# tiborcamargo/KinectPy

Hardware: AMD Instinct MI355X
Metric: Mpoints/sec end-to-end (unproject+filter+ICP), 4-sensor frame (higher is better)
Workload: dtype f64 decisions / f32 storage

## Files before the change

### kinectpy_amd/csrc/kpx_voxel.hip

```cpp
#include "kpx_voxelsteps.h"

namespace kpx {

template <bool NRM>
__global__ __launch_bounds__(256) void voxel_mean_kernel(StoredLoad load, int64_t n, const int32_t *__restrict__ vals, const int32_t *__restrict__ seg_start,
                                                         int32_t *__restrict__ d_count, const int32_t *__restrict__ err, float *__restrict__ opts,
                                                         float *__restrict__ ocol, float *__restrict__ onrm)
{
    const int32_t m_total = *d_count;
    if (blockIdx.x == 0 && threadIdx.x == 0 && *err) *d_count = KPX_ERR_RANGE;
    for (int64_t m = (int64_t)blockIdx.x * blockDim.x + threadIdx.x; m < m_total; m += (int64_t)gridDim.x * blockDim.x) {
        const int64_t s0 = seg_start[m], s1 = (m + 1 < m_total) ? seg_start[m + 1] : n;
        double sp[3] = { 0, 0, 0 }, sc[3] = { 0, 0, 0 }, sn[3] = { 0, 0, 0 };
        voxel_segment_sum<NRM>(vals, s0, s1, load, sp, sc, sn);
        voxel_write_row(sp, sc, (double)(s1 - s0), opts + 3 * m, (load.col && ocol) ? ocol + 3 * m : nullptr);
        if (NRM && onrm) {
            double nn = sqrt(fma(sn[2], sn[2], fma(sn[1], sn[1], sn[0] * sn[0])));
#pragma unroll
            for (int a = 0; a < 3; ++a) onrm[3 * m + a] = (float)(nn > 0 ? sn[a] / nn : sn[a]);
        }
    }
}
static int voxel_impl(const float *pts, const float *col, const float *nrm, int64_t n, double voxel, float *opts,
                      float *ocol, float *onrm, int32_t *d_count, Arena &a, hipStream_t st)
{
    VoxelScratch s;
    voxel_carve(a, n, kPlainCarve, &s);
    KPX_ARENA_CHECK(a);
    int rc = bbox_f32(pts, n, s.bbox, s.part, st);
    if (rc) return rc;
    KPX_HIP(hipMemsetAsync(s.err, 0, sizeof(int32_t), st));
    int nb = (int)(cdiv(n, 256) > 4096 ? 4096 : cdiv(n, 256));
    CloudSet<1> one;
    one.pts[0] = pts; one.off[0] = 0; one.off[1] = n; one.count = 1;
    hipLaunchKernelGGL((voxel_key_kernel<CloudSet<1>, StoredPoint, FixedKeys>), dim3(nb), dim3(256), 0, st, one, (const double *)s.bbox, voxel,
                       FixedKeys{ s.sort.keys_in, s.err }, s.sort.vals_in);
    rc = voxel_sort_and_heads<uint64_t>(s, n, 63, d_count, st);
    if (rc) return rc;
    const StoredLoad load = { pts, col, nrm, 0 };
    const auto mean_kernel = nrm ? &voxel_mean_kernel<true> : &voxel_mean_kernel<false>;
    hipLaunchKernelGGL(mean_kernel, dim3(nb), dim3(256), 0, st, load, n, (const int32_t *)s.sort.vals_out,
                       (const int32_t *)s.seg_start, d_count, (const int32_t *)s.err, opts, ocol, onrm);
    KPX_LAUNCH_CHECK();
    return KPX_OK;
}

constexpr int kVoxelBatchMax = 8;
constexpr int kVoxelBatchBboxBlocks = 64;
constexpr VoxelCarve kBatchCarve = { kVoxelBatchMax, kVoxelBatchBboxBlocks, true, true, 64 };
struct VoxelBatch : CloudSet<kVoxelBatchMax> {
    const float *col[kVoxelBatchMax];
    float *opts[kVoxelBatchMax];
    float *ocol[kVoxelBatchMax];
    int32_t morton;
};
static VoxelBatch voxel_batch_of(const float *const *h_pts, const float *const *h_col, const int64_t *h_n, float *const *h_opts, float *const *h_ocol,
                                 int first, int count, bool morton)
{
    VoxelBatch b;
    b.count = count;
    b.morton = morton ? 1 : 0;
    b.off[0] = 0;
    for (int i = 0; i < kVoxelBatchMax; ++i) {
        const bool on = i < count;
        b.pts[i] = on ? h_pts[first + i] : nullptr;
        b.col[i] = (on && h_col) ? h_col[first + i] : nullptr;
        b.opts[i] = on ? h_opts[first + i] : nullptr;
        b.ocol[i] = (on && h_col && h_ocol) ? h_ocol[first + i] : nullptr;
        b.off[i + 1] = b.off[i] + (on ? h_n[first + i] : 0);
    }
    return b;
}
__device__ __forceinline__ void voxel_batch_axis_bits(const double d[3], int bits[3])
{
#pragma unroll
    for (int a = 0; a < 3; ++a) {
        const unsigned long long m = (unsigned long long)d[a] - 1ull;
        int n = 1;
        while (n < 21 && (m >> n) != 0ull) ++n;
        bits[a] = n;
    }
}
__device__ __forceinline__ unsigned long long voxel_hcode(unsigned long long x, unsigned long long y, unsigned long long z, int bits)
{
    unsigned long long X[3] = { x, y, z };
    const unsigned long long M = 1ull << (bits - 1);
    for (unsigned long long Q = M; Q > 1ull; Q >>= 1) {
        const unsigned long long P = Q - 1ull;
#pragma unroll
        for (int i = 0; i < 3; ++i) {
            if (X[i] & Q) X[0] ^= P;
            else { const unsigned long long t = (X[0] ^ X[i]) & P; X[0] ^= t; X[i] ^= t; }
        }
    }
    X[1] ^= X[0];
    X[2] ^= X[1];
    unsigned long long t = 0ull;
    for (unsigned long long Q = M; Q > 1ull; Q >>= 1)
        if (X[2] & Q) t ^= Q - 1ull;
    X[0] ^= t; X[1] ^= t; X[2] ^= t;
    unsigned long long k = 0ull;
    for (int b = bits - 1; b >= 0; --b) {
#pragma unroll
        for (int i = 0; i < 3; ++i) k = (k << 1) | ((X[i] >> b) & 1ull);
    }
    return k;
}
__device__ __forceinline__ int voxel_hilbert_cube_bits(const int ab[3], int cb)
{
    const int top = ab[0] > ab[1] ? (ab[0] > ab[2] ? ab[0] : ab[2]) : (ab[1] > ab[2] ? ab[1] : ab[2]);
    const int low = ab[0] < ab[1] ? (ab[0] < ab[2] ? ab[0] : ab[2]) : (ab[1] < ab[2] ? ab[1] : ab[2]);
    const int passes = (ab[0] + ab[1] + ab[2] + cb + 7) / 8;
    for (int m = top; m > low; --m) {
        int n = 3 * m + cb;
#pragma unroll
        for (int a = 0; a < 3; ++a) n += ab[a] > m ? ab[a] - m : 0;
        if (n <= 64 && (n + 7) / 8 <= passes) return m;
    }
    return low;
}
__device__ __forceinline__ int voxel_hilbert_key_bits(const int ab[3], int m)
{
    int n = 3 * m;
#pragma unroll
    for (int a = 0; a < 3; ++a) n += ab[a] > m ? ab[a] - m : 0;
    return n;
}
__device__ __forceinline__ unsigned long long voxel_hilbert_key(unsigned long long x, unsigned long long y, unsigned long long z, const int ab[3], int m)
{
    const unsigned long long mask = (1ull << m) - 1ull;
    const int ey = ab[1] > m ? ab[1] - m : 0, ez = ab[2] > m ? ab[2] - m : 0;
    const unsigned long long hi = (((x >> m) << ey | (y >> m)) << ez) | (z >> m);
    return (hi << (3 * m)) | voxel_hcode(x & mask, y & mask, z & mask, m);
}
__device__ __forceinline__ void voxel_batch_dims(const VoxelBatch &b, const double *__restrict__ bbox, double voxel, double d[3], int *overflow)
{
    d[0] = d[1] = d[2] = 1.0;
    for (int c = 0; c < b.count; ++c) {
        if (b.off[c + 1] == b.off[c]) continue;
        double f[3];
        (void)voxel_cell(bbox + 8 * c + 3, bbox + 8 * c, voxel, f);
        for (int a = 0; a < 3; ++a) {
            const double e = f[a] + 1.0;
            if (e > d[a] && e < kVoxelAxisCells) d[a] = e;
        }
    }
    *overflow = ((double)b.count * d[0]) * (d[1] * d[2]) >= 18446744073709551616.0 ? 1 : 0;
}
__device__ __forceinline__ int voxel_batch_key_bits(const VoxelBatch &b, const double d[3], int overflow)
{
    int n = 64;
    if (!overflow && b.morton) {
        int cb = 0, ab[3];
        while ((1 << cb) < b.count) ++cb;
        voxel_batch_axis_bits(d, ab);
        n = voxel_hilbert_key_bits(ab, voxel_hilbert_cube_bits(ab, cb)) + cb;
        n = n < 1 ? 1 : (n > 64 ? 64 : n);
    } else if (!overflow) {
        const unsigned long long range = (((unsigned long long)b.count * (unsigned long long)d[0]) * (unsigned long long)d[1]) * (unsigned long long)d[2];
        n = 1;
        while (n < 64 && (range >> n) != 0ull) ++n;
    }
    return n;
}
__global__ void voxel_batch_bits_kernel(VoxelBatch b, const double *__restrict__ bbox, double voxel, int32_t *__restrict__ bits)
{
    double d[3];
    int overflow;
    voxel_batch_dims(b, bbox, voxel, d, &overflow);
    *bits = voxel_batch_key_bits(b, d, overflow);
}
template <class Key> struct BatchKeys {
    struct Grid {
        uint64_t DX, DY, DZ;
        int overflow, morton, ab[3], m;
    };
    Key *keys;
    int32_t *err, *bits_out;
    __device__ __forceinline__ Grid grid(const VoxelBatch &b, const double *__restrict__ bbox, double voxel) const
    {
        __shared__ double dims[3];
        __shared__ int overflow, axis_bits[3], cube_bits;
        if (threadIdx.x == 0) {
            double d[3];
            int ov;
            voxel_batch_dims(b, bbox, voxel, d, &ov);
            if (bits_out && blockIdx.x == 0) *bits_out = voxel_batch_key_bits(b, d, ov);
            dims[0] = d[0]; dims[1] = d[1]; dims[2] = d[2];
            int ab[3], cb = 0;
            voxel_batch_axis_bits(d, ab);
            axis_bits[0] = ab[0]; axis_bits[1] = ab[1]; axis_bits[2] = ab[2];
            while ((1 << cb) < b.count) ++cb;
            cube_bits = voxel_hilbert_cube_bits(ab, cb);
            overflow = (ov || (b.morton && voxel_hilbert_key_bits(ab, cube_bits) + cb > 64)) ? 1 : 0;
        }
        __syncthreads();
        return Grid{ (uint64_t)dims[0], (uint64_t)dims[1], (uint64_t)dims[2], overflow, b.morton, { axis_bits[0], axis_bits[1], axis_bits[2] }, cube_bits };
    }
    __device__ __forceinline__ void put(const Grid &g, const double *__restrict__ bbox, double voxel, int64_t i, int c, const double q[3]) const
    {
        double f[3];
        const bool bad = voxel_cell(q, bbox + 8 * c, voxel, f) || g.overflow;
        if (bad) { err[c] = 1; f[0] = f[1] = f[2] = 0.0; }
        if (g.morton)
            keys[i] = (Key)(((uint64_t)c << voxel_hilbert_key_bits(g.ab, g.m)) | voxel_hilbert_key((uint64_t)f[0], (uint64_t)f[1], (uint64_t)f[2], g.ab, g.m));
        else keys[i] = (Key)((((uint64_t)c * g.DX + (uint64_t)f[0]) * g.DY + (uint64_t)f[1]) * g.DZ + (uint64_t)f[2]);
    }
};
__global__ __launch_bounds__(64) void voxel_batch_locate_kernel(VoxelBatch b, const int32_t *__restrict__ seg_start, const int32_t *__restrict__ d_total,
                                                                const int32_t *__restrict__ err, int32_t *__restrict__ head, int32_t *__restrict__ d_counts)
{
    __shared__ int32_t h[kVoxelBatchMax + 1];
    const int c = threadIdx.x;
    const int32_t m = *d_total;
    if (c <= b.count) {
        int32_t lo = 0, hi = m;
        const int64_t want = b.off[c];
        while (lo < hi) {
            const int32_t mid = lo + (hi - lo) / 2;
            if (seg_start[mid] < want) lo = mid + 1; else hi = mid;
        }
        h[c] = c == b.count ? m : lo;
        head[c] = h[c];
    }
    __syncthreads();
    if (c < b.count) d_counts[c] = err[c] ? KPX_ERR_RANGE : h[c + 1] - h[c];
}
__global__ __launch_bounds__(256) void voxel_batch_mean_kernel(VoxelBatch b, const int32_t *__restrict__ vals, const int32_t *__restrict__ seg_start,
                                                               const int32_t *__restrict__ d_total, const int32_t *__restrict__ head)
{
    const int32_t m_total = *d_total;
    const int64_t total = b.off[b.count];
    for (int64_t m = (int64_t)blockIdx.x * blockDim.x + threadIdx.x; m < m_total; m += (int64_t)gridDim.x * blockDim.x) {
        const int64_t s0 = seg_start[m], s1 = (m + 1 < m_total) ? seg_start[m + 1] : total;
        const int c = b.cloud_of(s0);
        const StoredLoad load = { b.pts[c], b.col[c], nullptr, b.off[c] };
        double sp[3] = { 0, 0, 0 }, sc[3] = { 0, 0, 0 }, sn[3];
        voxel_segment_sum<false>(vals, s0, s1, load, sp, sc, sn);
        const int64_t o = m - head[c];
        voxel_write_row(sp, sc, (double)(s1 - s0), b.opts[c] + 3 * o, (load.col && b.ocol[c]) ? b.ocol[c] + 3 * o : nullptr);
    }
}

static int voxel_batch_impl(const VoxelBatch &b, double voxel, int32_t *d_counts, Arena &a, hipStream_t st, int spec_bits = 0,
                            int32_t *d_bits = nullptr)
{
    const int64_t total = b.off[b.count];
    VoxelScratch s;
    voxel_carve(a, total, kBatchCarve, &s);
    KPX_ARENA_CHECK(a);
    BoxDst boxes;
    for (int c = 0; c < kVoxelBatchMax; ++c) boxes.box[c] = s.bbox + 8 * c;
    boxes.err = s.err;
    hipLaunchKernelGGL((cloud_bbox_partial_kernel<VoxelBatch, StoredPoint, float, kVoxelBatchBboxBlocks>), dim3(kVoxelBatchBboxBlocks, b.count), dim3(256), 0, st, b, s.part);
    hipLaunchKernelGGL(cloud_bbox_final_kernel<kVoxelBatchBboxBlocks>, dim3(b.count), dim3(64), 0, st, (const double *)s.part, boxes);
    const int nb = (int)(cdiv(total, 256) > 4096 ? 4096 : cdiv(total, 256));
    int end_bit = 64;
    int32_t *bits_out = nullptr;
    if (spec_bits > 0 && d_bits) {
        bits_out = d_bits;
        end_bit = spec_bits > 64 ? 64 : spec_bits;
    } else if (total > (int64_t)128 * 1024) {
        int32_t *h_bits = static_cast<int32_t *>(thread_resources().pinned(kPinVoxelBits, sizeof(int32_t)));
        if (!h_bits) return KPX_ERR_HIP;
        hipLaunchKernelGGL(voxel_batch_bits_kernel, dim3(1), dim3(1), 0, st, b, s.bbox, voxel, s.head);
        KPX_HIP(hipMemcpyAsync(h_bits, s.head, sizeof(int32_t), hipMemcpyDeviceToHost, st));
        if (d_bits) KPX_HIP(hipMemcpyAsync(d_bits, s.head, sizeof(int32_t), hipMemcpyDefault, st));
        KPX_HIP(hipStreamSynchronize(st));
        end_bit = *h_bits < 1 ? 1 : (*h_bits > 64 ? 64 : *h_bits);
    } else if (d_bits) {
        hipLaunchKernelGGL(voxel_batch_bits_kernel, dim3(1), dim3(1), 0, st, b, s.bbox, voxel, d_bits);
    }
    int rc;
    if (end_bit <= 32) {
        hipLaunchKernelGGL((voxel_key_kernel<VoxelBatch, StoredPoint, BatchKeys<uint32_t>>), dim3(nb), dim3(256), 0, st, b, (const double *)s.bbox, voxel,
                           BatchKeys<uint32_t>{ reinterpret_cast<uint32_t *>(s.sort.keys_in), s.err, bits_out }, s.sort.vals_in);
        rc = voxel_sort_and_heads<uint32_t>(s, total, end_bit, s.d_total, st);
    } else {
        hipLaunchKernelGGL((voxel_key_kernel<VoxelBatch, StoredPoint, BatchKeys<uint64_t>>), dim3(nb), dim3(256), 0, st, b, (const double *)s.bbox, voxel,
                           BatchKeys<uint64_t>{ s.sort.keys_in, s.err, bits_out }, s.sort.vals_in);
        rc = voxel_sort_and_heads<uint64_t>(s, total, end_bit, s.d_total, st);
    }
    if (rc) return rc;
    hipLaunchKernelGGL(voxel_batch_locate_kernel, dim3(1), dim3(64), 0, st, b, s.seg_start, s.d_total, s.err, s.head, d_counts);
    hipLaunchKernelGGL(voxel_batch_mean_kernel, dim3(nb), dim3(256), 0, st, b, s.sort.vals_out, s.seg_start, s.d_total, s.head);
    KPX_LAUNCH_CHECK();
    return KPX_OK;
}

constexpr int kFuseMax = 16;
constexpr int kFuseBboxBlocks = 32;
constexpr VoxelCarve kFuseCarve = { kFuseMax, kFuseBboxBlocks, false, true, 63 };
struct FuseBatch : CloudSet<kFuseMax> {
    const float *col[kFuseMax];
    double T[kFuseMax][12];
    const double *dT[kFuseMax];
};
__global__ __launch_bounds__(64) void fuse_bbox_final_kernel(const double *__restrict__ part, int rows, double *__restrict__ bbox, int32_t *__restrict__ err)
{
    const int lane = lane_id();
    double v[6] = { INFINITY, INFINITY, INFINITY, -INFINITY, -INFINITY, -INFINITY };
    for (int r = lane; r < rows; r += 64) {
#pragma unroll
        for (int a = 0; a < 3; ++a) { v[a] = fmin(v[a], part[(int64_t)r * 6 + a]); v[3 + a] = fmax(v[3 + a], part[(int64_t)r * 6 + 3 + a]); }
    }
    box_wave_fold(v, v + 3);
    if (lane == 0) {
        for (int a = 0; a < 6; ++a) bbox[a] = v[a];
        *err = 0;
    }
}
__device__ __forceinline__ int fuse_key_bits(const double *__restrict__ bbox, double voxel, double d[3], bool *sane_out)
{
    (void)voxel_cell(bbox + 3, bbox, voxel, d);
#pragma unroll
    for (int a = 0; a < 3; ++a) d[a] += 1.0;
    const bool sane = d[0] >= 1.0 && d[1] >= 1.0 && d[2] >= 1.0 && d[0] < kVoxelAxisCells && d[1] < kVoxelAxisCells && d[2] < kVoxelAxisCells;
    int bits = 64;
    if (sane && d[0] * d[1] * d[2] < 18446744073709551616.0) {
        const unsigned long long range = (unsigned long long)d[0] * (unsigned long long)d[1] * (unsigned long long)d[2];
        bits = 1;
        while (bits < 64 && (range >> bits) != 0ull) ++bits;
    }
    *sane_out = sane;
    return bits;
}
__global__ void fuse_bits_kernel(const double *__restrict__ bbox, double voxel, int32_t *__restrict__ bits_out)
{
    double d[3];
    bool sane;
    *bits_out = fuse_key_bits(bbox, voxel, d, &sane);
}
struct ExtentKeys32 {
    struct Grid {
        double d[3];
        unsigned long long DY, DZ;
    };
    uint32_t *keys;
    int32_t *bits_out;
    template <class Set> __device__ __forceinline__ Grid grid(const Set &, const double *__restrict__ bbox, double voxel) const
    {
        Grid g;
        bool sane;
        const int bits = fuse_key_bits(bbox, voxel, g.d, &sane);
        if (blockIdx.x == 0 && threadIdx.x == 0) *bits_out = bits;
        g.DY = sane ? (unsigned long long)g.d[1] : 1ull;
        g.DZ = sane ? (unsigned long long)g.d[2] : 1ull;
        return g;
    }
    __device__ __forceinline__ void put(const Grid &g, const double *__restrict__ bbox, double voxel, int64_t i, int, const double q[3]) const
    {
        double f[3];
        if (voxel_cell(q, bbox, voxel, f, g.d)) f[0] = f[1] = f[2] = 0.0;
        keys[i] = (uint32_t)(((unsigned long long)f[0] * g.DY + (unsigned long long)f[1]) * g.DZ + (unsigned long long)f[2]);
    }
};
struct MovedLoad {
    using Coord = double;
    const FuseBatch &b;
    __device__ __forceinline__ bool has_col() const { return true; }
    __device__ __forceinline__ void operator()(int64_t p, double v[3], float c[3], float *) const
    {
        const int cl = b.cloud_of(p);
        const int64_t j = p - b.off[cl];
        MovedPoint()(b, cl, j, v);
        const float *col = b.col[cl];
#pragma unroll
        for (int a = 0; a < 3; ++a) c[a] = col ? col[3 * j + a] : 0.0f;
    }
};
__global__ __launch_bounds__(256) void fuse_mean_kernel(FuseBatch b, const int32_t *__restrict__ vals, const int32_t *__restrict__ seg_start,
                                                        int32_t *__restrict__ d_count, const int32_t *__restrict__ err, float *__restrict__ opts,
                                                        float *__restrict__ ocol)
{
    const int32_t m_total = *d_count;
    if (blockIdx.x == 0 && threadIdx.x == 0 && *err) *d_count = KPX_ERR_RANGE;
    const int64_t total = b.off[b.count];
    for (int64_t m = (int64_t)blockIdx.x * blockDim.x + threadIdx.x; m < m_total; m += (int64_t)gridDim.x * blockDim.x) {
        const int64_t s0 = seg_start[m], s1 = (m + 1 < m_total) ? seg_start[m + 1] : total;
        double sp[3] = { 0, 0, 0 }, sc[3] = { 0, 0, 0 }, sn[3];
        voxel_segment_sum<false>(vals, s0, s1, MovedLoad{ b }, sp, sc, sn);
        voxel_write_row(sp, sc, (double)(s1 - s0), opts + 3 * m, ocol ? ocol + 3 * m : nullptr);
    }
}
static int fuse_voxel_impl(const FuseBatch &b, double voxel, float *opts, float *ocol, int32_t *d_count, Arena &a, hipStream_t st, int spec_bits = 0,
                           int32_t *d_bits = nullptr)
{
    const int64_t total = b.off[b.count];
    VoxelScratch s;
    voxel_carve(a, total, kFuseCarve, &s);
    KPX_ARENA_CHECK(a);
    hipLaunchKernelGGL((cloud_bbox_partial_kernel<FuseBatch, MovedPoint, double, kFuseBboxBlocks>), dim3(kFuseBboxBlocks, b.count), dim3(256), 0, st, b, s.part);
    hipLaunchKernelGGL(fuse_bbox_final_kernel, dim3(1), dim3(64), 0, st, s.part, b.count * kFuseBboxBlocks, s.bbox, s.err);
    const int nb = (int)(cdiv(total, 256) > 4096 ? 4096 : cdiv(total, 256));
    int rc;
    if (spec_bits > 0 && spec_bits <= 32 && d_bits && total <= kRadixMaxPairs) {
        hipLaunchKernelGGL((voxel_key_kernel<FuseBatch, MovedPoint, ExtentKeys32>), dim3(nb), dim3(256), 0, st, b, (const double *)s.bbox, voxel,
                           ExtentKeys32{ reinterpret_cast<uint32_t *>(s.sort.keys_in), d_bits }, s.sort.vals_in);
        rc = voxel_sort_and_heads<uint32_t>(s, total, spec_bits, d_count, st);
    } else {
        if (d_bits) hipLaunchKernelGGL(fuse_bits_kernel, dim3(1), dim3(1), 0, st, s.bbox, voxel, d_bits);
        hipLaunchKernelGGL((voxel_key_kernel<FuseBatch, MovedPoint, FixedKeys>), dim3(nb), dim3(256), 0, st, b, (const double *)s.bbox, voxel,
                           FixedKeys{ s.sort.keys_in, s.err }, s.sort.vals_in);
        rc = voxel_sort_and_heads<uint64_t>(s, total, 63, d_count, st);
    }
    if (rc) return rc;
    hipLaunchKernelGGL(fuse_mean_kernel, dim3(nb), dim3(256), 0, st, b, s.sort.vals_out, s.seg_start, d_count, s.err, opts, ocol);
    KPX_LAUNCH_CHECK();
    return KPX_OK;
}
}

using namespace kpx;

KPX_EXPORT size_t kpx_fuse_voxel_workspace_bytes(int64_t total)
{
    Arena a(nullptr, 0);
    VoxelScratch s;
    voxel_carve(a, total, kFuseCarve, &s);
    return a.off;
}
KPX_EXPORT int kpx_fuse_voxel_downsample(int32_t count, const float *const *h_pts, const float *const *h_col, const int64_t *h_n,
                                         const double *h_T, double voxel, float *opts, float *ocol, int32_t *d_count, void *ws,
                                         size_t ws_bytes, void *stream)
{
    return kpx::fuse_voxel_downsample_dev(count, h_pts, h_col, h_n, h_T, nullptr, voxel, opts, ocol, d_count, ws, ws_bytes, stream, 0, nullptr);
}
int kpx::fuse_voxel_downsample_dev(int32_t count, const float *const *h_pts, const float *const *h_col, const int64_t *h_n, const double *h_T,
                                   const double *const *h_dT, double voxel, float *opts, float *ocol, int32_t *d_count, void *ws, size_t ws_bytes,
                                   void *stream, int spec_bits, int32_t *d_bits)
{
    KPX_REQUIRE(voxel > 0.0, "voxel_size <= 0");
    KPX_REQUIRE(count >= 1 && count <= kFuseMax, "kpx_fuse_voxel_downsample: 1 .. %d clouds", kFuseMax);
    KPX_REQUIRE(h_pts && h_n && h_T && d_count && ws, "kpx_fuse_voxel_downsample: null pointer");
    hipStream_t st = (hipStream_t)stream;
    FuseBatch b;
    b.count = count;
    b.off[0] = 0;
    bool any_col = false, all_col = true;
    for (int i = 0; i < kFuseMax; ++i) {
        const bool on = i < count;
        if (on) {
            KPX_REQUIRE(h_n[i] >= 0 && (h_n[i] == 0 || h_pts[i]), "kpx_fuse_voxel_downsample: bad cloud %d", i);
            if (h_n[i] > 0) { const bool hc = h_col && h_col[i]; any_col |= hc; all_col &= hc; }
        }
        b.pts[i] = on ? h_pts[i] : nullptr;
        b.col[i] = (on && h_col) ? h_col[i] : nullptr;
        b.off[i + 1] = b.off[i] + (on ? h_n[i] : 0);
        for (int k = 0; k < 12; ++k) b.T[i][k] = on ? h_T[16 * i + k] : 0.0;
        b.dT[i] = (on && h_dT) ? h_dT[i] : nullptr;
    }
    const int64_t total = b.off[count];
    KPX_REQUIRE(total < ((int64_t)1 << 31), "kpx_fuse_voxel_downsample: bad size");
    KPX_REQUIRE(!ocol || !any_col || all_col, "kpx_fuse_voxel_downsample: colours on some clouds only");
    if (total == 0) { KPX_HIP(hipMemsetAsync(d_count, 0, sizeof(int32_t), st)); return KPX_OK; }
    KPX_REQUIRE(opts, "kpx_fuse_voxel_downsample: null pointer");
    Arena a(ws, ws_bytes);
    return fuse_voxel_impl(b, voxel, opts, (any_col && all_col) ? ocol : nullptr, d_count, a, st, spec_bits, d_bits);
}

KPX_EXPORT size_t kpx_voxel_workspace_bytes(int64_t n)
{
    return kpx_voxel_batch_workspace_bytes(1, &n);
}
KPX_EXPORT int kpx_voxel_downsample(const float *pts, const float *col, const float *nrm, int64_t n, double voxel,
                                    float *opts, float *ocol, float *onrm, int32_t *d_count, void *ws, size_t ws_bytes,
                                    void *stream)
{
    KPX_REQUIRE(voxel > 0.0, "voxel_size <= 0");
    KPX_REQUIRE(n >= 0 && n < ((int64_t)1 << 31), "kpx_voxel_downsample: bad size");
    KPX_REQUIRE(d_count && ws, "kpx_voxel_downsample: null pointer");
    hipStream_t st = (hipStream_t)stream;
    if (n == 0) { KPX_HIP(hipMemsetAsync(d_count, 0, sizeof(int32_t), st)); return KPX_OK; }
    KPX_REQUIRE(pts && opts, "kpx_voxel_downsample: null pointer");
    Arena a(ws, ws_bytes);
    static const bool single_batch = [] { const char *e = getenv("KPX_VOXEL_SINGLE"); return !(e && e[0] == '0'); }();
    if (!nrm && single_batch) {
        return voxel_batch_impl(voxel_batch_of(&pts, &col, &n, &opts, col ? &ocol : nullptr, 0, 1, false), voxel, d_count, a, st);
    }
    return voxel_impl(pts, col, nrm, n, voxel, opts, ocol, onrm, d_count, a, st);
}

KPX_EXPORT size_t kpx_voxel_batch_workspace_bytes(int32_t count, const int64_t *h_n)
{
    if (count < 1 || !h_n) return 0;
    Arena a(nullptr, 0), one(nullptr, 0);
    VoxelScratch s;
    int64_t total = 0;
    for (int i = 0; i < count; ++i) {
        voxel_carve(a, h_n[i], kPlainCarve, &s);
        total += h_n[i] > 0 ? h_n[i] : 0;
    }
    voxel_carve(one, total, kBatchCarve, &s);
    return a.off > one.off ? a.off : one.off;
}
KPX_EXPORT int kpx_voxel_downsample_batch(int32_t count, const float *const *h_pts, const float *const *h_col, const int64_t *h_n,
                                          double voxel, float *const *h_opts, float *const *h_ocol, int32_t *d_counts, void *ws,
                                          size_t ws_bytes, void *stream)
{
    return kpx::voxel_downsample_batch_spec(count, h_pts, h_col, h_n, voxel, h_opts, h_ocol, d_counts, ws, ws_bytes, stream, 0, nullptr, false);
}
int kpx::voxel_downsample_batch_spec(int32_t count, const float *const *h_pts, const float *const *h_col, const int64_t *h_n, double voxel,
                                     float *const *h_opts, float *const *h_ocol, int32_t *d_counts, void *ws, size_t ws_bytes, void *stream,
                                     int spec_bits, int32_t *d_bits, bool morton)
{
    KPX_REQUIRE(voxel > 0.0, "voxel_size <= 0");
    KPX_REQUIRE(count >= 1 && count <= 64 && h_pts && h_n && h_opts && d_counts && ws, "kpx_voxel_downsample_batch: bad arguments");
    for (int i = 0; i < count; ++i)
        KPX_REQUIRE(h_n[i] >= 0 && h_n[i] < ((int64_t)1 << 31) && (h_n[i] == 0 || (h_pts[i] && h_opts[i])),
                    "kpx_voxel_downsample_batch: bad cloud %d", i);
    hipStream_t st = (hipStream_t)stream;
    int64_t total = 0;
    for (int i = 0; i < count; ++i) total += h_n[i];
    if (count <= kVoxelBatchMax && total > 0 && total < ((int64_t)1 << 31)) {
        Arena one(ws, ws_bytes);
        return voxel_batch_impl(voxel_batch_of(h_pts, h_col, h_n, h_opts, h_ocol, 0, count, morton), voxel, d_counts, one, st, spec_bits, d_bits);
    }
    if (d_bits) KPX_HIP(hipMemsetAsync(d_bits, 0, sizeof(int32_t), st));
    if (count > kVoxelBatchMax && total > 0) {
        int gstart[65], ng = 0;
        bool ok = true;
        for (int i = 0; i < count;) {
            gstart[ng++] = i;
            int64_t gt = 0;
            int gc = 0;
            while (i < count && gc < kVoxelBatchMax) { gt += h_n[i]; ++gc; ++i; }
            ok = ok && gt < ((int64_t)1 << 31);
        }
        gstart[ng] = count;
        if (ok) {
            for (int g = 0; g < ng; ++g) {
                const int g0 = gstart[g], gc = gstart[g + 1] - g0;
                int64_t gt = 0;
                for (int i = 0; i < gc; ++i) gt += h_n[g0 + i];
                if (gt == 0) { KPX_HIP(hipMemsetAsync(d_counts + g0, 0, (size_t)gc * sizeof(int32_t), st)); continue; }
                Arena one(ws, ws_bytes);
                const int grc = voxel_batch_impl(voxel_batch_of(h_pts, h_col, h_n, h_opts, h_ocol, g0, gc, false), voxel, d_counts + g0, one, st);
                if (grc) return grc;
            }
            return KPX_OK;
        }
    }
    LaneSet *ln = nullptr;
    int rc = lanes_get(&ln);
    if (rc) return rc;
    const int used = count < kLaneCount ? count : kLaneCount;
    rc = lanes_fork(ln, st, used);
    if (rc) return rc;
    Arena a(ws, ws_bytes);
    for (int i = 0; i < count && !rc; ++i) {
        hipStream_t ls = ln->s[i % kLaneCount];
        if (h_n[i] == 0) { rc = hipMemsetAsync(d_counts + i, 0, sizeof(int32_t), ls) == hipSuccess ? KPX_OK : fail(KPX_ERR_HIP, "memset failed"); continue; }
        rc = voxel_impl(h_pts[i], h_col ? h_col[i] : nullptr, nullptr, h_n[i], voxel, h_opts[i], (h_col && h_ocol) ? h_ocol[i] : nullptr, nullptr,
                        d_counts + i, a, ls);
    }
    const int jrc = lanes_join(ln, st, used);
    return rc ? rc : jrc;
}
```

### kinectpy_amd/csrc/kpx_voxelsteps.h

```cpp
#pragma once
#include "kpx_cloudset.h"
#include "kpx_internal.h"
#include "kpx_sort.h"

namespace kpx {

constexpr double kVoxelAxisCells = 2097152.0;
__device__ __forceinline__ bool voxel_cell_at(const double q[3], const double org[3], double voxel, double f[3], const double *own = nullptr)
{
#pragma unroll
    for (int a = 0; a < 3; ++a) f[a] = floor((q[a] - org[a]) / voxel);
    if (!(f[0] >= 0.0) || !(f[1] >= 0.0) || !(f[2] >= 0.0)) return true;
    if (own) return !(f[0] < own[0]) || !(f[1] < own[1]) || !(f[2] < own[2]);
    return f[0] >= kVoxelAxisCells || f[1] >= kVoxelAxisCells || f[2] >= kVoxelAxisCells;
}
__device__ __forceinline__ bool voxel_cell(const double q[3], const double *__restrict__ bbox, double voxel, double f[3], const double *own = nullptr)
{
    const double org[3] = { bbox[0] - voxel * 0.5, bbox[1] - voxel * 0.5, bbox[2] - voxel * 0.5 };
    return voxel_cell_at(q, org, voxel, f, own);
}
template <class Set, class Src, class Pack>
__global__ __launch_bounds__(256) void voxel_key_kernel(Set b, const double *__restrict__ bbox, double voxel, Pack pack, int32_t *__restrict__ vals)
{
    const typename Pack::Grid g = pack.grid(b, bbox, voxel);
    const int64_t total = b.off[b.count];
    for (int64_t i = (int64_t)blockIdx.x * blockDim.x + threadIdx.x; i < total; i += (int64_t)gridDim.x * blockDim.x) {
        const int c = b.cloud_of(i);
        double q[3];
        Src()(b, c, i - b.off[c], q);
        pack.put(g, bbox, voxel, i, c, q);
        vals[i] = (int32_t)i;
    }
}
struct FixedKeys {
    struct Grid {};
    uint64_t *keys;
    int32_t *err;
    template <class Set> __device__ __forceinline__ Grid grid(const Set &, const double *, double) const { return Grid(); }
    __device__ __forceinline__ void put(const Grid &, const double *__restrict__ bbox, double voxel, int64_t i, int, const double q[3]) const
    {
        double f[3];
        if (voxel_cell(q, bbox, voxel, f)) { *err = 1; f[0] = f[1] = f[2] = 0.0; }
        keys[i] = ((uint64_t)f[0] << 42) | ((uint64_t)f[1] << 21) | (uint64_t)f[2];
    }
};

template <class Key> struct HeadPredT {
    const Key *keys;
    __device__ bool operator()(int64_t s, int) const { return s == 0 || keys[s] != keys[s - 1]; }
};
struct HeadEmit {
    int32_t *seg_start;
    __device__ void operator()(int64_t s, int, int32_t dst) const { seg_start[dst] = (int32_t)s; }
};

template <bool NRM, class Load>
__device__ __forceinline__ void voxel_segment_sum(const int32_t *__restrict__ vals, int64_t s0, int64_t s1, const Load &load, double sp[3],
                                                  double sc[3], double sn[3])
{
    for (int64_t s = s0; s < s1; s += 8) {
        const int cnt = (int)(s1 - s < 8 ? s1 - s : 8);
        int64_t p[8];
#pragma unroll
        for (int k = 0; k < 8; ++k) p[k] = k < cnt ? vals[s + k] : -1;
        typename Load::Coord vp[8][3];
        float vc[8][3], vn[8][3];
#pragma unroll
        for (int k = 0; k < 8; ++k) {
            if (p[k] < 0) continue;
            load(p[k], vp[k], vc[k], vn[k]);
        }
#pragma unroll
        for (int k = 0; k < 8; ++k) {
            if (p[k] < 0) continue;
#pragma unroll
            for (int a = 0; a < 3; ++a) {
                sp[a] += (double)vp[k][a];
                if (load.has_col()) sc[a] += (double)vc[k][a];
                if (NRM) sn[a] += (double)vn[k][a];
            }
        }
    }
}
__device__ __forceinline__ void voxel_write_row(const double sp[3], const double sc[3], double cn, float *__restrict__ opts, float *__restrict__ ocol)
{
#pragma unroll
    for (int a = 0; a < 3; ++a) {
        opts[a] = (float)(sp[a] / cn);
        if (ocol) ocol[a] = (float)(sc[a] / cn);
    }
}
struct StoredLoad {
    using Coord = float;
    const float *pts, *col, *nrm;
    int64_t base;
    __device__ __forceinline__ bool has_col() const { return col != nullptr; }
    __device__ __forceinline__ void operator()(int64_t p, float v[3], float c[3], float n[3]) const
    {
        const int64_t j = p - base;
#pragma unroll
        for (int a = 0; a < 3; ++a) {
            v[a] = pts[3 * j + a];
            if (col) c[a] = col[3 * j + a];
            if (nrm) n[a] = nrm[3 * j + a];
        }
    }
};

using VoxelSort = DeviceSort<uint64_t, true, kSortDefault32>;
struct VoxelScratch {
    int32_t *seg_start, *counts, *err, *head, *d_total;
    double *part, *bbox;
    VoxelSort sort;
    char *counts_end;
};
struct VoxelCarve {
    int clouds, bbox_blocks;
    bool per_cloud, keys32;
    int end_bit;
};
static void voxel_carve(Arena &a, int64_t total, const VoxelCarve &v, VoxelScratch *s)
{
    const size_t nn = (size_t)(total > 0 ? total : 1);
    s->seg_start = a.get<int32_t>(nn);
    s->err = a.get<int32_t>(v.per_cloud ? v.clouds : 1);
    s->head = v.per_cloud ? a.get<int32_t>(v.clouds + 1) : nullptr;
    s->d_total = v.per_cloud ? a.get<int32_t>(1) : nullptr;
    s->part = a.get<double>((size_t)v.clouds * v.bbox_blocks * 6);
    s->bbox = a.get<double>((size_t)(v.per_cloud ? v.clouds : 1) * 8);
    SortOptions o;
    if (v.keys32) { o.radix = kRadixAndVendor; o.tmp_floor = dsort_view32_bytes(total); }
    dsort_carve(a, total, v.end_bit, o, &s->sort);
    s->counts = a.get<int32_t>((size_t)compact_ws_ints(total));
    s->counts_end = reinterpret_cast<char *>(s->counts + (size_t)compact_ws_ints(total));
}

template <class Key>
static int voxel_sort_and_heads(const VoxelScratch &s, int64_t total, int end_bit, int32_t *d_heads, hipStream_t st)
{
    const bool narrow = sizeof(Key) == 4;
    const DeviceSortView32 v = dsort_view32(s.sort);
    const bool cleared = narrow && dsort_by_radix(v, total);
    const int rc = narrow ? dsort_run(v, total, end_bit, st, s.counts_end) : dsort_run(s.sort, total, end_bit, st);
    if (rc) return rc;
    return compact(HeadPredT<Key>{ reinterpret_cast<const Key *>(s.sort.keys_out) }, HeadEmit{ s.seg_start }, total, 1, s.counts, d_heads, st, cleared);
}

constexpr VoxelCarve kPlainCarve = { 1, kBboxBlocks, false, false, 63 };

}
```

Baseline: 2517.

## Stage voxel segment gathers through shared-memory tiles for cooperative mean reduction

Replaces the one-thread-per-voxel mean loops with a block-tiled scheme. Each block takes a window of sorted positions and finds its voxel range with a wave-parallel lower bound. Threads then gather the points coalesced by sorted index into shared memory, and each thread sums its voxel from LDS. This is meant to remove the load imbalance and uncoalesced serial gathers when voxel sizes vary, at the cost of extra barriers, shared-memory use and a per-window binary search. Grid sizes are now derived from the per-load tile chunk instead of a fixed per-thread count.

Result: no change. 2534 (median of 6 runs) (+0.6%).

```diff
diff --git a/kinectpy_amd/csrc/kpx_voxel.hip b/kinectpy_amd/csrc/kpx_voxel.hip
--- a/kinectpy_amd/csrc/kpx_voxel.hip
+++ b/kinectpy_amd/csrc/kpx_voxel.hip
@@ -9,17 +9,14 @@
 {
     const int32_t m_total = *d_count;
     if (blockIdx.x == 0 && threadIdx.x == 0 && *err) *d_count = KPX_ERR_RANGE;
-    for (int64_t m = (int64_t)blockIdx.x * blockDim.x + threadIdx.x; m < m_total; m += (int64_t)gridDim.x * blockDim.x) {
-        const int64_t s0 = seg_start[m], s1 = (m + 1 < m_total) ? seg_start[m + 1] : n;
-        double sp[3] = { 0, 0, 0 }, sc[3] = { 0, 0, 0 }, sn[3] = { 0, 0, 0 };
-        voxel_segment_sum<NRM>(vals, s0, s1, load, sp, sc, sn);
+    voxel_tile_means<NRM>(vals, seg_start, m_total, n, load, [&](int64_t m, int64_t s0, int64_t s1, const double sp[3], const double sc[3], const double sn[3]) {
         voxel_write_row(sp, sc, (double)(s1 - s0), opts + 3 * m, (load.col && ocol) ? ocol + 3 * m : nullptr);
         if (NRM && onrm) {
             double nn = sqrt(fma(sn[2], sn[2], fma(sn[1], sn[1], sn[0] * sn[0])));
 #pragma unroll
             for (int a = 0; a < 3; ++a) onrm[3 * m + a] = (float)(nn > 0 ? sn[a] / nn : sn[a]);
         }
-    }
+    });
 }
 static int voxel_impl(const float *pts, const float *col, const float *nrm, int64_t n, double voxel, float *opts,
                       float *ocol, float *onrm, int32_t *d_count, Arena &a, hipStream_t st)
@@ -39,7 +36,7 @@
     if (rc) return rc;
     const StoredLoad load = { pts, col, nrm, 0 };
     const auto mean_kernel = nrm ? &voxel_mean_kernel<true> : &voxel_mean_kernel<false>;
-    hipLaunchKernelGGL(mean_kernel, dim3(nb), dim3(256), 0, st, load, n, (const int32_t *)s.sort.vals_out,
+    hipLaunchKernelGGL(mean_kernel, dim3(voxel_tile_blocks<StoredLoad>(n)), dim3(256), 0, st, load, n, (const int32_t *)s.sort.vals_out,
                        (const int32_t *)s.seg_start, d_count, (const int32_t *)s.err, opts, ocol, onrm);
     KPX_LAUNCH_CHECK();
     return KPX_OK;
@@ -226,20 +223,26 @@
     __syncthreads();
     if (c < b.count) d_counts[c] = err[c] ? KPX_ERR_RANGE : h[c + 1] - h[c];
 }
+struct BatchLoad {
+    using Coord = float;
+    static constexpr int kTileChunk = StoredLoad::kTileChunk;
+    const VoxelBatch &b;
+    __device__ __forceinline__ StoredLoad at(int64_t i) const
+    {
+        const int c = b.cloud_of(i);
+        return StoredLoad{ b.pts[c], b.col[c], nullptr, b.off[c] };
+    }
+};
 __global__ __launch_bounds__(256) void voxel_batch_mean_kernel(VoxelBatch b, const int32_t *__restrict__ vals, const int32_t *__restrict__ seg_start,
                                                                const int32_t *__restrict__ d_total, const int32_t *__restrict__ head)
 {
     const int32_t m_total = *d_total;
     const int64_t total = b.off[b.count];
-    for (int64_t m = (int64_t)blockIdx.x * blockDim.x + threadIdx.x; m < m_total; m += (int64_t)gridDim.x * blockDim.x) {
-        const int64_t s0 = seg_start[m], s1 = (m + 1 < m_total) ? seg_start[m + 1] : total;
+    voxel_tile_means<false>(vals, seg_start, m_total, total, BatchLoad{ b }, [&](int64_t m, int64_t s0, int64_t s1, const double sp[3], const double sc[3], const double *) {
         const int c = b.cloud_of(s0);
-        const StoredLoad load = { b.pts[c], b.col[c], nullptr, b.off[c] };
-        double sp[3] = { 0, 0, 0 }, sc[3] = { 0, 0, 0 }, sn[3];
-        voxel_segment_sum<false>(vals, s0, s1, load, sp, sc, sn);
         const int64_t o = m - head[c];
-        voxel_write_row(sp, sc, (double)(s1 - s0), b.opts[c] + 3 * o, (load.col && b.ocol[c]) ? b.ocol[c] + 3 * o : nullptr);
-    }
+        voxel_write_row(sp, sc, (double)(s1 - s0), b.opts[c] + 3 * o, (b.col[c] && b.ocol[c]) ? b.ocol[c] + 3 * o : nullptr);
+    });
 }
 
 static int voxel_batch_impl(const VoxelBatch &b, double voxel, int32_t *d_counts, Arena &a, hipStream_t st, int spec_bits = 0,
@@ -283,7 +286,7 @@
     }
     if (rc) return rc;
     hipLaunchKernelGGL(voxel_batch_locate_kernel, dim3(1), dim3(64), 0, st, b, s.seg_start, s.d_total, s.err, s.head, d_counts);
-    hipLaunchKernelGGL(voxel_batch_mean_kernel, dim3(nb), dim3(256), 0, st, b, s.sort.vals_out, s.seg_start, s.d_total, s.head);
+    hipLaunchKernelGGL(voxel_batch_mean_kernel, dim3(voxel_tile_blocks<BatchLoad>(total)), dim3(256), 0, st, b, s.sort.vals_out, s.seg_start, s.d_total, s.head);
     KPX_LAUNCH_CHECK();
     return KPX_OK;
 }
@@ -357,8 +360,10 @@
 };
 struct MovedLoad {
     using Coord = double;
+    static constexpr int kTileChunk = 512;
     const FuseBatch &b;
     __device__ __forceinline__ bool has_col() const { return true; }
+    __device__ __forceinline__ const MovedLoad &at(int64_t) const { return *this; }
     __device__ __forceinline__ void operator()(int64_t p, double v[3], float c[3], float *) const
     {
         const int cl = b.cloud_of(p);
@@ -376,12 +381,9 @@
     const int32_t m_total = *d_count;
     if (blockIdx.x == 0 && threadIdx.x == 0 && *err) *d_count = KPX_ERR_RANGE;
     const int64_t total = b.off[b.count];
-    for (int64_t m = (int64_t)blockIdx.x * blockDim.x + threadIdx.x; m < m_total; m += (int64_t)gridDim.x * blockDim.x) {
-        const int64_t s0 = seg_start[m], s1 = (m + 1 < m_total) ? seg_start[m + 1] : total;
-        double sp[3] = { 0, 0, 0 }, sc[3] = { 0, 0, 0 }, sn[3];
-        voxel_segment_sum<false>(vals, s0, s1, MovedLoad{ b }, sp, sc, sn);
+    voxel_tile_means<false>(vals, seg_start, m_total, total, MovedLoad{ b }, [&](int64_t m, int64_t s0, int64_t s1, const double sp[3], const double sc[3], const double *) {
         voxel_write_row(sp, sc, (double)(s1 - s0), opts + 3 * m, ocol ? ocol + 3 * m : nullptr);
-    }
+    });
 }
 static int fuse_voxel_impl(const FuseBatch &b, double voxel, float *opts, float *ocol, int32_t *d_count, Arena &a, hipStream_t st, int spec_bits = 0,
                            int32_t *d_bits = nullptr)
@@ -405,7 +407,7 @@
         rc = voxel_sort_and_heads<uint64_t>(s, total, 63, d_count, st);
     }
     if (rc) return rc;
-    hipLaunchKernelGGL(fuse_mean_kernel, dim3(nb), dim3(256), 0, st, b, s.sort.vals_out, s.seg_start, d_count, s.err, opts, ocol);
+    hipLaunchKernelGGL(fuse_mean_kernel, dim3(voxel_tile_blocks<MovedLoad>(total)), dim3(256), 0, st, b, s.sort.vals_out, s.seg_start, d_count, s.err, opts, ocol);
     KPX_LAUNCH_CHECK();
     return KPX_OK;
 }
diff --git a/kinectpy_amd/csrc/kpx_voxelsteps.h b/kinectpy_amd/csrc/kpx_voxelsteps.h
--- a/kinectpy_amd/csrc/kpx_voxelsteps.h
+++ b/kinectpy_amd/csrc/kpx_voxelsteps.h
@@ -92,9 +92,11 @@
 }
 struct StoredLoad {
     using Coord = float;
+    static constexpr int kTileChunk = 1024;
     const float *pts, *col, *nrm;
     int64_t base;
     __device__ __forceinline__ bool has_col() const { return col != nullptr; }
+    __device__ __forceinline__ const StoredLoad &at(int64_t) const { return *this; }
     __device__ __forceinline__ void operator()(int64_t p, float v[3], float c[3], float n[3]) const
     {
         const int64_t j = p - base;
@@ -106,6 +108,117 @@
         }
     }
 };
+
+__device__ __forceinline__ uint32_t voxel_head_lower_bound(const int32_t *__restrict__ seg_start, uint32_t m_total, uint32_t want)
+{
+    const uint32_t lane = threadIdx.x & 63;
+    uint32_t lo = 0, hi = m_total;
+    while (lo < hi) {
+        const uint32_t step = (hi - lo + 63) / 64, idx = lo + (lane + 1) * step - 1;
+        const bool below = idx < hi && (uint32_t)seg_start[idx] < want;
+        const uint32_t c = __popcll(__ballot(below));
+        const uint32_t top = lo + (c + 1) * step - 1;
+        lo += c * step;
+        hi = top < hi ? top : hi;
+        lo = lo < hi ? lo : hi;
+    }
+    return lo;
+}
+
+constexpr int kVoxelTileGroup = 256;
+template <class Loads> static int voxel_tile_blocks(int64_t total)
+{
+    const int64_t nb = cdiv(total, (int64_t)Loads::kTileChunk);
+    return (int)(nb > 4096 ? 4096 : (nb < 1 ? 1 : nb));
+}
+template <bool NRM, class Loads, class Emit>
+__device__ __forceinline__ void voxel_tile_means(const int32_t *__restrict__ vals, const int32_t *__restrict__ seg_start, int32_t m_total, int64_t total,
+                                                 const Loads &loads, const Emit &emit)
+{
+    using Coord = typename Loads::Coord;
+    constexpr int G = kVoxelTileGroup, C = Loads::kTileChunk, K = C / G;
+    static_assert(C % G == 0 && (C & (C - 1)) == 0, "a chunk is a power of two and a whole number of positions per thread");
+    __shared__ Coord tp[3][C];
+    __shared__ float tc[3][C], tn[NRM ? 3 : 1][NRM ? C : 1];
+    __shared__ uint32_t window_m[2];
+    const uint32_t tid = threadIdx.x;
+    if (m_total <= 0) return;
+    const uint32_t M = (uint32_t)m_total, end = (uint32_t)total;
+    for (uint32_t w0 = blockIdx.x * C; w0 < end; w0 += gridDim.x * C) {
+        if (tid < 128) {
+            const uint32_t f = voxel_head_lower_bound(seg_start, M, w0 + (tid >> 6) * C);
+            if ((tid & 63) == 0) window_m[tid >> 6] = f;
+        }
+        __syncthreads();
+        const uint32_t mlo = window_m[0], mhi = window_m[1];
+        __syncthreads();
+        const uint32_t rend = mhi < M ? (uint32_t)seg_start[mhi] : end;
+        for (uint32_t m0 = mlo; m0 < mhi; m0 += G) {
+            const uint32_t m = m0 + tid;
+            const uint32_t r0 = seg_start[m0], r1 = (m0 + G < mhi) ? (uint32_t)seg_start[m0 + G] : rend;
+            const bool own = m < mhi;
+            const uint32_t s0 = own ? seg_start[m] : 0, s1 = !own ? 0 : (m + 1 < mhi) ? (uint32_t)seg_start[m + 1] : rend;
+            const bool col = own && loads.at(s0).has_col();
+            double sp[3] = { 0, 0, 0 }, sc[3] = { 0, 0, 0 }, sn[3] = { 0, 0, 0 };
+            for (uint32_t cb = r0; cb < r1; cb += C) {
+                int32_t pv[K];
+#pragma unroll
+                for (int k = 0; k < K; ++k) pv[k] = cb + k * G + tid < r1 ? vals[cb + k * G + tid] : -1;
+                Coord vp[K][3];
+                float vc[K][3], vn[K][3];
+                bool hc[K];
+#pragma unroll
+                for (int k = 0; k < K; ++k) {
+                    hc[k] = false;
+                    if (pv[k] < 0) continue;
+                    const auto &ld = loads.at(pv[k]);
+                    hc[k] = ld.has_col();
+                    ld(pv[k], vp[k], vc[k], vn[k]);
+                }
+#pragma unroll
+                for (int k = 0; k < K; ++k) {
+                    if (pv[k] < 0) continue;
+#pragma unroll
+                    for (int a = 0; a < 3; ++a) {
+                        tp[a][k * G + tid] = vp[k][a];
+                        if (hc[k]) tc[a][k * G + tid] = vc[k][a];
+                        if constexpr (NRM) tn[a][k * G + tid] = vn[k][a];
+                    }
+                }
+                __syncthreads();
+                const uint32_t ce = cb + C < r1 ? cb + C : r1;
+                const uint32_t lo = s0 > cb ? s0 : cb, hi = s1 < ce ? s1 : ce;
+                for (uint32_t s = lo; s < hi; s += 4) {
+                    const uint32_t cnt = hi - s < 4 ? hi - s : 4;
+                    Coord xp[4][3];
+                    float xc[4][3], xn[4][3];
+#pragma unroll
+                    for (int k = 0; k < 4; ++k) {
+                        const uint32_t i = (s - cb + k) & (C - 1);
+#pragma unroll
+                        for (int a = 0; a < 3; ++a) {
+                            xp[k][a] = tp[a][i];
+                            if (col) xc[k][a] = tc[a][i];
+                            if constexpr (NRM) xn[k][a] = tn[a][i];
+                        }
+                    }
+#pragma unroll
+                    for (int k = 0; k < 4; ++k) {
+                        if (k >= cnt) continue;
+#pragma unroll
+                        for (int a = 0; a < 3; ++a) {
+                            sp[a] += (double)xp[k][a];
+                            if (col) sc[a] += (double)xc[k][a];
+                            if (NRM) sn[a] += (double)xn[k][a];
+                        }
+                    }
+                }
+                __syncthreads();
+            }
+            if (own) emit(m, s0, s1, sp, sc, sn);
+        }
+    }
+}
 
 using VoxelSort = DeviceSort<uint64_t, true, kSortDefault32>;
 struct VoxelScratch {
```
